# yanyan-li/Structure-SLAM-PointLine

Measured on AMD Instinct MI355X. Metric: front-end frames/sec (ORB+LSD extract+match) 640x480 @1000kp/200ln, higher is better.
Workload: dtype u8; 1 GPU; BASELINE configs[2]: 640x480 ORB(1000kp,8 levels)+LSD/LBD(<=200 lines) extract + Hamming match vs previous frame, inputs resident in HBM; batch_per_gpu=12288, global_batch=12288, unique_frames=64, streams=point branch and line branch on two HIP streams, parallelism=single GPU

## Files before the change

### structure-slam-pointline_amd/csrc/orb.hip

```cpp
#include "common.h"
#include "camera.h"
#include <cmath>
#include <algorithm>

using namespace sslam;

namespace {

constexpr int MAX_LEVELS = 16;
constexpr int MAX_ROOTS = 64;
constexpr int EDGE = 19;
constexpr int MINB = 16;
constexpr int HALF_PATCH = 15;

struct LevelInfo {
    int w, h, pitch;
    unsigned off;
    int cellBeg, nCells;
    int candOff, candCap;
    int nfeat;
    int selOff, selCap;
    int nIni;
    float hX;
    int W, H;
    float scale;
    float size;
    int tabX, tabY;
    float rcpGroups;
};

struct Plan {
    int nlevels;
    int nCellsFrame, candFrame, selFrame;
    unsigned blurPack0, blurPack1;
    const uint4* blurToep;
    int blurTapSum;
    size_t pyrFrame;
    const uint8_t* img0; size_t img0Stride; int img0Pitch;
    int maxCellW, maxCellH, maxCellsLevel, maxNodeCap;
    LevelInfo L[MAX_LEVELS];
};

struct CellInfo {
    short level, x0, y0, x1, y1;
    short pad;
    int candOff;
    unsigned magic, gmagic;
};

__device__ __forceinline__ const uint8_t* level_image(const Plan& P, const uint8_t* __restrict__ pyr, size_t pyrFrame, int b, int level, int& pitch) {
    if (level == 0 && P.img0) { pitch = P.img0Pitch; return P.img0 + (size_t)b * P.img0Stride; }
    pitch = P.L[level].pitch;
    return pyr + (size_t)b * pyrFrame + P.L[level].off;
}

__device__ const signed char kPat[1024] = {
#include "orb_pattern.inc"
};
__constant__ int kUmax[16];
typedef short s16x2 __attribute__((ext_vector_type(2)));
__device__ __forceinline__ s16x2 as_s16x2(unsigned v) { return __builtin_bit_cast(s16x2, v); }
__device__ __forceinline__ unsigned as_u32(s16x2 v) { return __builtin_bit_cast(unsigned, v); }
__constant__ unsigned kDiscMask[31 * 8];

__global__ void k_copy_level0(const uint8_t* __restrict__ in, size_t pitch, size_t imageStride,
                              uint8_t* __restrict__ pyr, size_t pyrFrame, int w, int h, int dpitch) {
    const int b = blockIdx.z;
    const int y = blockIdx.y;
    const int x = (blockIdx.x * blockDim.x + threadIdx.x) * 16;
    if (x >= w) return;
    const uint8_t* s = in + (size_t)b * imageStride + (size_t)y * pitch + x;
    uint8_t* d = pyr + (size_t)b * pyrFrame + (size_t)y * dpitch + x;
// ... 90 lines not shown
        cd = cd && ((r[k] < v - minTh) || (r[k + 8] < v - minTh));
    }
    if (!(cb || cd)) return 0;
    auto network = [&](int (&d)[16], int sg) -> int {
#pragma unroll
        for (int k = 0; k < 16; ++k) d[k] = (d[k] - v) ^ sg;
        const int d0 = d[0], d1 = d[1];
#pragma unroll
        for (int k = 0; k < 14; ++k) d[k] = min(min(d[k], d[k + 1]), d[k + 2]);
        d[14] = min(min(d[14], d[15]), d0);
        d[15] = min(min(d[15], d0), d1);
        int A = min(min(d[0], d[3]), d[6]);
#pragma unroll
        for (int k = 1; k < 16; ++k) A = max(A, min(min(d[k], d[(k + 3) & 15]), d[(k + 6) & 15]));
        return A - sg;
    };
    int best = max(0, network(r, cd ? -1 : 0));
    const bool both = cb && cd;
    if (__builtin_amdgcn_ballot_w64(both)) {
        const uint8_t* c2 = c;
        asm volatile("" : "+v"(c2));
        int q[16];
        q[0] = c2[3 * tp];      q[1] = c2[3 * tp + 1];   q[2] = c2[2 * tp + 2];   q[3] = c2[tp + 3];
        q[4] = c2[3];           q[5] = c2[-tp + 3];      q[6] = c2[-2 * tp + 2];  q[7] = c2[-3 * tp + 1];
        q[8] = c2[-3 * tp];     q[9] = c2[-3 * tp - 1];  q[10] = c2[-2 * tp - 2]; q[11] = c2[-tp - 3];
        q[12] = c2[-3];         q[13] = c2[tp - 3];      q[14] = c2[2 * tp - 2];  q[15] = c2[3 * tp - 1];
        const int b2 = network(q, 0);
        if (both) best = max(best, b2);
    }
    int s = best - 1;
    return s >= minTh ? s : 0;
}

constexpr int FAST_LIST_CAP = 832;

static inline int fast_tile_pitch(int maxW) { return (maxW + 6 + 3 + 7) & ~3; }
static inline int fast_score_pitch(int maxW) { return maxW + 1; }
static inline size_t fast_score_bytes(int maxW, int maxH) { return (((size_t)(maxH + 2) * fast_score_pitch(maxW) + 1) + 3) & ~(size_t)3; }
static inline size_t fast_lds_bytes(int maxW, int maxH) {
    return (size_t)(maxH + 6) * fast_tile_pitch(maxW) + fast_score_bytes(maxW, maxH) + sizeof(unsigned short) * FAST_LIST_CAP;
}

__global__ __launch_bounds__(64) void k_fast_cells(const uint8_t* __restrict__ pyr, size_t pyrFrame, Plan P,
                                                   const CellInfo* __restrict__ cells,
                                                   unsigned* __restrict__ cand, int* __restrict__ cellCount,
                                                   int iniTh, int minTh, int tileP, int scP) {
    extern __shared__ __align__(16) uint8_t lds[];
    const int b = blockIdx.y, per = gridDim.x >> 3;
    const int cellId = (((blockIdx.x & 7) + b) & 7) * per + (blockIdx.x >> 3);
    if (cellId >= P.nCellsFrame) return;
    const int lane = threadIdx.x;
    const CellInfo ci = cells[cellId];
    const LevelInfo& L = P.L[ci.level];
    const int cw = ci.x1 - ci.x0, ch = ci.y1 - ci.y0;
    uint8_t* tile = lds;
    uint8_t* sc = tile + (P.maxCellH + 6) * tileP;
    int pitch;
    const uint8_t* img = level_image(P, pyr, pyrFrame, b, ci.level, pitch);
    const int ax = (ci.x0 - 3) & ~3, off = (ci.x0 - 3) - ax;
    const int ndw = (off + cw + 6 + 3) >> 2, th = ch + 6;
    {
        const __amdgpu_buffer_rsrc_t rs = __builtin_amdgcn_make_buffer_rsrc((void*)(img + (size_t)(ci.y0 - 3) * pitch + ax), 0, 0x7FFFFFFF, 0x00020000);
        const int q0 = lane & 15;
        for (int ry = lane >> 4; ry < th; ry += 4) {
            const int rowOff = __mul24(ry, pitch);
            for (int q = q0; q < ndw; q += 16) ((unsigned*)(tile + ry * tileP))[q] = __builtin_amdgcn_raw_buffer_load_b32(rs, rowOff + 4 * q, 0, 0);
        }
    }
    for (int i = lane; i < (((ch + 2) * scP + 1 + 3) >> 2); i += 64) ((unsigned*)sc)[i] = 0;
    __syncthreads();
    const unsigned magic = ci.magic;
    unsigned short* clist = (unsigned short*)(sc + (((P.maxCellH + 2) * scP + 1 + 3) & ~3));
    int ncl = 0;
    bool dense = false;
    const int T0 = off + 3;
    const int gmin = T0 >> 2, ng = ((T0 + cw - 1) >> 2) - gmin + 1;
    const unsigned gmagic = ci.gmagic;
    const int nitems = ch * ng;
    for (int it0 = 0;;) {
        const s16x2 th2 = {(short)minTh, (short)minTh};
        int la = lane;
        asm volatile("" : "+v"(la));
        for (ncl = 0; it0 < nitems; it0 += 64) {
            const int it = it0 + la;
            unsigned flags = 0;
            int py = 0, g = 0;
            if (it < nitems) {
                py = (int)(__umul24((unsigned)it, gmagic) >> 19);
                g = gmin + (it - __mul24(py, ng));
                const int rowN = __mul24(py, tileP);
                const unsigned* rc = (const unsigned*)(tile + rowN + 3 * tileP) + g;
                const unsigned c1 = rc[0], c0 = rc[-1], c2 = rc[1];
                const unsigned n4 = ((const unsigned*)(tile + rowN))[g], s4 = ((const unsigned*)(tile + rowN + 6 * tileP))[g];
                unsigned res = 0;
#pragma unroll
                for (int h = 0; h < 2; ++h) {
                    const unsigned wsel = h == 0 ? 0x0c020c00u : 0x0c030c01u;
                    const s16x2 v = as_s16x2(__builtin_amdgcn_perm(0u, c1, wsel));
                    const s16x2 rn = as_s16x2(__builtin_amdgcn_perm(0u, n4, wsel)), rs = as_s16x2(__builtin_amdgcn_perm(0u, s4, wsel));
                    const s16x2 re = as_s16x2(__builtin_amdgcn_perm(c2, c1, h == 0 ? 0x0c050c03u : 0x0c060c04u)), rw = as_s16x2(__builtin_amdgcn_perm(c1, c0, h == 0 ? 0x0c030c01u : 0x0c040c02u));
                    const s16x2 vp = v + th2, vm = v - th2;
                    const s16x2 mxV = __builtin_elementwise_max(rn, rs), mnV = __builtin_elementwise_min(rn, rs);
                    const s16x2 mxH = __builtin_elementwise_max(re, rw), mnH = __builtin_elementwise_min(re, rw);
                    const unsigned bright = as_u32(vp - __builtin_elementwise_min(mxV, mxH));
                    const unsigned dark = as_u32(__builtin_elementwise_max(mnV, mnH) - vm);
                    const unsigned m = (bright | dark) & 0x80008000u;
                    res |= m >> (15 - h);
                }
                flags = (res & 3u) | ((res >> 14) & 12u);
                const int px0 = 4 * g - T0;
                flags &= (0xFu << max(0, -px0)) & (0xFu >> max(0, px0 + 4 - cw));
            }
            const int cntf = __popc(flags);
            const int incl = wave_incl_scan(cntf);
            const int tot = __builtin_amdgcn_readlane(incl, 63);
            if (ncl + tot > FAST_LIST_CAP) { dense = true; break; }
            int pos = ncl + incl - cntf;
            const int ibase = __mul24(py, cw) + 4 * g - T0;
#pragma unroll
            for (int k = 0; k < 4; ++k) if (flags & (1u << k)) clist[pos++] = (unsigned short)(ibase + k);
            ncl += tot;
        }
        __syncthreads();
        for (int j = lane; j < ncl; j += 64) {
            const int i = clist[j];
            const int py = (int)(__umul24((unsigned)i, magic) >> 19), px = i - __mul24(py, cw);
            const int s = fast_score16(tile + __mul24(py + 3, tileP) + (off + px + 3), tileP, minTh);
            if (s) sc[__mul24(py + 1, scP) + (px + 1)] = (uint8_t)s;
        }
        __syncthreads();
        if (it0 >= nitems) break;
    }
    auto keep_code = [&](const uint8_t* c) -> int {
        const int s = c[0];
        const int n0 = c[-1], n1 = c[1], n2 = c[-scP - 1], n3 = c[-scP], n4 = c[-scP + 1], n5 = c[scP - 1], n6 = c[scP], n7 = c[scP + 1];
        const int mx = max(max(max(n0, n1), max(n2, n3)), max(max(n4, n5), max(n6, n7)));
        return (s > mx) ? (s >= iniTh ? 2 : 1) : 0;
    };
    unsigned* out = cand + (size_t)b * P.candFrame + ci.candOff;
    int cnt20 = 0, n = 0;
    if (!dense) {
        for (int j0 = 0; j0 < ncl; j0 += 64) {
            const int j = j0 + lane;
            int cde = 0;
            if (j < ncl) {
                const int i = clist[j];
                const int py = (int)(__umul24((unsigned)i, magic) >> 19), px = i - __mul24(py, cw);
                cde = keep_code(sc + __mul24(py + 1, scP) + (px + 1));
                clist[j] = (unsigned short)(i | (cde << 13));
            }
            cnt20 += __popcll(__ballot(cde == 2));
        }
        __syncthreads();
        const int need = cnt20 > 0 ? 2 : 1;
        for (int j0 = 0; j0 < ncl; j0 += 64) {
            const int j = j0 + lane;
            int e = 0;
            if (j < ncl) e = clist[j];
            const bool keep = (e >> 13) >= need;
            unsigned long long m = __ballot(keep);
            if (keep) {
                const int i = e & 0x1FFF;
                const int py = (int)(__umul24((unsigned)i, magic) >> 19), px = i - __mul24(py, cw);
                int s = sc[__mul24(py + 1, scP) + (px + 1)];
                out[n + mbcnt(m)] = ((unsigned)s << 24) | ((unsigned)(ci.y0 + py - MINB) << 12) | (unsigned)(ci.x0 + px - MINB);
            }
            n += __popcll(m);
        }
    } else {
        const int npx = __mul24(ch, cw);
        for (int i0 = 0; i0 < npx; i0 += 64) {
            const int i = i0 + lane;
            int cde = 0;
            if (i < npx) {
                const int py = (int)(__umul24((unsigned)i, magic) >> 19), px = i - __mul24(py, cw);
                cde = keep_code(sc + __mul24(py + 1, scP) + (px + 1));
            }
            cnt20 += __popcll(__ballot(cde == 2));
        }
        const int need = cnt20 > 0 ? 2 : 1;
        for (int i0 = 0; i0 < npx; i0 += 64) {
            const int i = i0 + lane;
            bool keep = false;
            int py = 0, px = 0;
            if (i < npx) {
                py = (int)(__umul24((unsigned)i, magic) >> 19); px = i - __mul24(py, cw);
                keep = keep_code(sc + __mul24(py + 1, scP) + (px + 1)) >= need;
            }
            unsigned long long m = __ballot(keep);
            if (keep) {
                int s = sc[__mul24(py + 1, scP) + (px + 1)];
                out[n + mbcnt(m)] = ((unsigned)s << 24) | ((unsigned)(ci.y0 + py - MINB) << 12) | (unsigned)(ci.x0 + px - MINB);
            }
            n += __popcll(m);
        }
    }
    if (lane == 0) cellCount[(size_t)b * P.nCellsFrame + cellId] = n;
}

struct OctLds {
    int* pre;
    unsigned* box0;
    unsigned* box1;
    unsigned* start;
    int* count;
    unsigned* links;
    unsigned long long* expA;
    unsigned long long* expB;
};

#define NIL 0xFFFFu

__global__ __launch_bounds__(64) void k_octree(const unsigned* __restrict__ cand, const int* __restrict__ cellCount,
                                               const CellInfo* __restrict__ cells, unsigned* __restrict__ bufA,
                                               unsigned* __restrict__ bufB, unsigned* __restrict__ sel,
                                               int* __restrict__ selCount, Plan P, int NC, int NCp2) {
    extern __shared__ __align__(16) uint8_t lds[];
    const int b = blockIdx.y, level = (int)((blockIdx.x + b + (b >> 3) + (b >> 6) + (b >> 9)) % gridDim.x), lane = threadIdx.x;
    const LevelInfo& L = P.L[level];
    OctLds S;
    S.expA = (unsigned long long*)lds;
    S.expB = S.expA + NCp2;
    S.pre = (int*)(S.expB + NCp2);
    S.box0 = (unsigned*)(S.pre + P.maxCellsLevel + 1);
    S.box1 = S.box0 + NC;
    S.start = S.box1 + NC;
    S.count = (int*)(S.start + NC);
    S.links = (unsigned*)(S.count + NC);

    const int nc = L.nCells;
// ... 414 lines not shown
            default: w = 0xFFFFFFFFu; break;
        }
        ((unsigned*)kpOut)[((size_t)b * cap + outIdx) * 7 + lane] = w;
    }
}

__global__ __launch_bounds__(256) void k_orb_status(const int* __restrict__ selCount, int nlevels, int nframes, int cap, int* __restrict__ status) {
    __shared__ int cnt, first;
    if (threadIdx.x == 0) { cnt = 0; first = 0x7FFFFFFF; }
    __syncthreads();
    for (int b = threadIdx.x; b < nframes; b += 256) {
        int t = 0;
        for (int l = 0; l < nlevels; ++l) t += selCount[(size_t)b * nlevels + l];
        if (t > cap) { atomicAdd(&cnt, 1); atomicMin(&first, b); }
    }
    __syncthreads();
    if (threadIdx.x == 0) { status[0] = cnt; status[1] = first; status[2] = 0; status[3] = 0x7FFFFFFF; }
}

}

struct sslam_orb {
    sslam_ctx* ctx;
    int nfeatures, nlevels, iniTh, minTh;
    float scaleFactorF;
    double scaleFactor;
    std::vector<float> scale, invScale, sigma2, invSigma2;
    std::vector<int> perLevel;
    int umax[16];
    int planW = 0, planH = 0;
    Plan plan;
    const uint8_t* lastImg0 = nullptr; size_t lastImg0Pitch = 0, lastImg0Stride = 0; bool lastInPlace = false;
    std::vector<CellInfo> cells;
    std::vector<short> tabs;
    DevBuf dCells, dTabs, dPyr, dCellCount, dCand, dBufA, dBufB, dSel, dSelCount;
    DevBuf dImg, dKp, dDesc, dCounts;
    HostPinned hImg, hOut;
    int wsFrames = 0;
    int lastFrames = 0;
    int lastN = -1;
    bool constsUploaded = false;
    int blurVariant = 0;
    hipEvent_t gateEvent = nullptr;
    bool hasCamera = false; sslam_camera camera{};
    DevBuf dToep; int toepVariant = -1, toepSum = 0;
};

static inline int cvRoundF(float v) { return (int)lrintf(v); }

static std::vector<int> blur_taps_340(int n, double sigma) {
    std::vector<float> k(n); double sum = 0; const double s2 = -0.5 / (sigma * sigma);
    for (int i = 0; i < n; ++i) { const double x = i - (n - 1) * 0.5; k[i] = (float)std::exp(s2 * x * x); sum += k[i]; }
    sum = 1. / sum;
    std::vector<int> t(n);
    for (int i = 0; i < n; ++i) { k[i] = (float)(k[i] * sum); t[i] = (int)lrint((double)k[i] * 256.0); }
    return t;
}
static std::vector<int> blur_taps_q8(int n, double sigma) {
    std::vector<double> k(n);
    double sum = 0, s2 = -0.5 / (sigma * sigma);
    for (int i = 0; i < n; ++i) { double x = i - (n - 1) * 0.5; k[i] = std::exp(s2 * x * x); sum += k[i]; }
    std::vector<int> t(n);
    double err = 0; long isum = 0;
    for (int i = 0; i < n / 2; ++i) {
        double adj = k[i] / sum * 256.0 + err;
        int v = (int)lrint(adj);
        err = adj - v; t[i] = t[n - 1 - i] = v; isum += v;
    }
// ... 92 lines not shown
                o->tabs.push_back((short)cvRoundF((1.f - fx) * 2048));
                o->tabs.push_back((short)cvRoundF(fx * 2048));
                o->tabs.push_back(0);
            }
            L.tabY = (int)o->tabs.size() / 4;
            for (int dy = 0; dy < L.h; ++dy) {
                float fy = (float)((dy + 0.5) * sy_ - 0.5);
                int sy = (int)std::floor(fy);
                fy -= sy;
                o->tabs.push_back((short)sy);
                o->tabs.push_back((short)cvRoundF((1.f - fy) * 2048));
                o->tabs.push_back((short)cvRoundF(fy * 2048));
                o->tabs.push_back(0);
            }
            while ((o->tabs.size() / 4) % 4) o->tabs.insert(o->tabs.end(), 4, (short)0);
        }
    }
    {
        int lvl = 0;
        for (int l = 1; l < o->nlevels; ++l) if (P.L[l].selCap > P.L[lvl].selCap) lvl = l;
        int NC, NCp2; size_t lds;
        octree_lds(P, NC, NCp2, lds);
        if (NC > 0xFFFF) {
            set_error("nfeatures %d: level %d would give the quadtree %d node slots (limit %d: 16-bit slot numbers)", o->nfeatures, lvl, NC, 0xFFFF); return SSLAM_ERR_UNSUPPORTED;
        }
        int ldsMax = 0;
        SSLAM_HIP(hipDeviceGetAttribute(&ldsMax, hipDeviceAttributeMaxSharedMemoryPerBlock, o->ctx->device));
        if (lds > (size_t)ldsMax) {
            set_error("nfeatures %d: level %d (%d keypoints) needs %zu bytes of LDS for the quadtree, the device allows %d", o->nfeatures, lvl, P.L[lvl].nfeat, lds, ldsMax); return SSLAM_ERR_UNSUPPORTED;
        }
    }
    P.pyrFrame = (off + 16 + 255) & ~(size_t)255;
    P.nCellsFrame = (int)o->cells.size();
    P.candFrame = std::max(candOff, 1);
    P.selFrame = selOff;
    if (o->dCells.ensure(std::max<size_t>(o->cells.size(), 1) * sizeof(CellInfo)) != SSLAM_OK) return SSLAM_ERR_HIP;
    if (o->dTabs.ensure(std::max<size_t>(o->tabs.size(), 1) * sizeof(short)) != SSLAM_OK) return SSLAM_ERR_HIP;
    if (!o->cells.empty()) SSLAM_HIP(hipMemcpy(o->dCells.p, o->cells.data(), o->cells.size() * sizeof(CellInfo), hipMemcpyHostToDevice));
    if (!o->tabs.empty()) SSLAM_HIP(hipMemcpy(o->dTabs.p, o->tabs.data(), o->tabs.size() * sizeof(short), hipMemcpyHostToDevice));
    o->planW = w; o->planH = h;
    o->wsFrames = 0;
    return SSLAM_OK;
}

static int ensure_workspace(sslam_orb* o, int nframes) {
    if (nframes <= o->wsFrames) return SSLAM_OK;
    const Plan& P = o->plan;
    int rc;
    if ((rc = o->dPyr.ensure(P.pyrFrame * nframes))) return rc;
    if ((rc = o->dCellCount.ensure(sizeof(int) * (size_t)std::max(P.nCellsFrame, 1) * nframes))) return rc;
    if ((rc = o->dCand.ensure(sizeof(unsigned) * (size_t)P.candFrame * nframes))) return rc;
    if ((rc = o->dBufA.ensure(sizeof(unsigned) * (size_t)P.candFrame * nframes))) return rc;
    if ((rc = o->dBufB.ensure(sizeof(unsigned) * (size_t)P.candFrame * nframes))) return rc;
    if ((rc = o->dSel.ensure(sizeof(unsigned) * (size_t)P.selFrame * nframes))) return rc;
    if ((rc = o->dSelCount.ensure(sizeof(int) * (size_t)P.nlevels * nframes))) return rc;
    o->wsFrames = nframes;
    return SSLAM_OK;
}

extern "C" int sslam_orb_create(sslam_ctx* ctx, int nfeatures, float scaleFactor, int nlevels, int iniTh, int minTh, sslam_orb** out) {
    if (!ctx || !out || nlevels < 1 || nlevels > MAX_LEVELS || nfeatures < 0 || !(scaleFactor > 1.0f) || minTh < 1 || iniTh < minTh || iniTh > 255) {
        set_error("sslam_orb_create: invalid arguments"); return SSLAM_ERR_INVALID;
    }
    sslam_orb* o = new sslam_orb();
    o->ctx = ctx; o->nfeatures = nfeatures; o->nlevels = nlevels; o->iniTh = iniTh; o->minTh = minTh;
    o->scaleFactorF = scaleFactor; o->scaleFactor = (double)scaleFactor;
    o->scale.resize(nlevels); o->sigma2.resize(nlevels); o->invScale.resize(nlevels); o->invSigma2.resize(nlevels);
    o->scale[0] = 1.0f; o->sigma2[0] = 1.0f;
    for (int i = 1; i < nlevels; ++i) { o->scale[i] = (float)(o->scale[i - 1] * o->scaleFactor); o->sigma2[i] = o->scale[i] * o->scale[i]; }
    for (int i = 0; i < nlevels; ++i) { o->invScale[i] = 1.0f / o->scale[i]; o->invSigma2[i] = 1.0f / o->sigma2[i]; }
    o->perLevel.resize(nlevels);
    float factor = (float)(1.0f / o->scaleFactor);
    float nDesired = nfeatures * (1 - factor) / (1 - (float)std::pow((double)factor, (double)nlevels));
    int sum = 0;
    for (int l = 0; l < nlevels - 1; ++l) { o->perLevel[l] = cvRoundF(nDesired); sum += o->perLevel[l]; nDesired *= factor; }
    o->perLevel[nlevels - 1] = std::max(nfeatures - sum, 0);
    {
        int v, v0, vmax = (int)std::floor(HALF_PATCH * std::sqrt(2.f) / 2 + 1);
        int vmin = (int)std::ceil(HALF_PATCH * std::sqrt(2.f) / 2);
        const double hp2 = HALF_PATCH * HALF_PATCH;
        for (v = 0; v <= vmax; ++v) o->umax[v] = (int)lrint(std::sqrt(hp2 - v * v));
        for (v = HALF_PATCH, v0 = 0; v >= vmin; --v) { while (o->umax[v0] == o->umax[v0 + 1]) ++v0; o->umax[v] = v0; ++v0; }
    }
    *out = o;
    return SSLAM_OK;
}

extern "C" int sslam_orb_set_blur_variant(sslam_orb* o, int variant) {
    if (!o || (variant != 0 && variant != 1)) { set_error("sslam_orb_set_blur_variant: invalid arguments"); return SSLAM_ERR_INVALID; }
    std::lock_guard<std::recursive_mutex> lk(o->ctx->mu);
    o->blurVariant = variant;
    return SSLAM_OK;
}

extern "C" int sslam_orb_destroy(sslam_orb* o) {
    if (!o) return SSLAM_OK;
    (void)hipSetDevice(o->ctx->device);
    (void)hipStreamSynchronize(o->ctx->stream);
    DevBuf* bufs[] = {&o->dCells, &o->dTabs, &o->dPyr, &o->dCellCount, &o->dCand, &o->dBufA, &o->dBufB, &o->dSel, &o->dSelCount, &o->dImg, &o->dKp, &o->dDesc, &o->dCounts, &o->dToep};
    for (DevBuf* b : bufs) b->release();
    o->hImg.release(); o->hOut.release();
    delete o;
    return SSLAM_OK;
}

extern "C" int sslam_orb_get_scales(const sslam_orb* o, float* scale, float* inv_scale, float* sigma2, float* inv_sigma2, int32_t* per_level) {
    if (!o) return SSLAM_ERR_INVALID;
    for (int i = 0; i < o->nlevels; ++i) {
        if (scale) scale[i] = o->scale[i];
        if (inv_scale) inv_scale[i] = o->invScale[i];
        if (sigma2) sigma2[i] = o->sigma2[i];
        if (inv_sigma2) inv_sigma2[i] = o->invSigma2[i];
        if (per_level) per_level[i] = o->perLevel[i];
    }
    return SSLAM_OK;
}

extern "C" int sslam_orb_set_gate_event(sslam_orb* o, void* hip_event) {
    if (!o) { set_error("sslam_orb_set_gate_event: null handle"); return SSLAM_ERR_INVALID; }
    std::lock_guard<std::recursive_mutex> lk(o->ctx->mu);
    o->gateEvent = (hipEvent_t)hip_event;
    return SSLAM_OK;
}

extern "C" int sslam_orb_max_keypoints(const sslam_orb* o) {
    if (!o) return SSLAM_ERR_INVALID;
    int n = 0;
    for (int l = 0; l < o->nlevels; ++l) n += std::max(o->perLevel[l] + 3, 4 * 8 + 1);
    return n;
}

static int orb_prepare(sslam_orb* o, int w, int h, int nframes, hipStream_t st) {
// ... 31 lines not shown
                unsigned w = 0;
                for (int k = 0; k < 4; ++k) { const int u = 4 * m + k - 15; if (std::abs(u) <= o->umax[std::abs(r - 15)]) w |= 0xFFu << (8 * k); }
                mask[r * 8 + m] = w;
            }
        SSLAM_HIP(hipMemcpyToSymbol(HIP_SYMBOL(kDiscMask), mask, sizeof(mask)));
        o->constsUploaded = true;
    }
    if (nframes > o->wsFrames) { SSLAM_HIP(hipStreamSynchronize(st)); }
    return ensure_workspace(o, nframes);
}

static int orb_front(sslam_orb* o, Plan& P, const uint8_t* d_images, int w, int h, size_t pitch, size_t image_stride, int nframes, hipStream_t st) {
    uint8_t* pyr = o->dPyr.as<uint8_t>();
    const bool inPlace = ((uintptr_t)d_images & 3) == 0 && (pitch & 3) == 0 && (image_stride & 3) == 0 && pitch <= 0x7FFFFFFF &&
                         (pitch == (size_t)w || image_stride >= pitch * (size_t)h);
    P.img0 = inPlace ? d_images : nullptr; P.img0Stride = image_stride; P.img0Pitch = (int)pitch;
    o->lastImg0 = d_images; o->lastImg0Pitch = pitch; o->lastImg0Stride = image_stride; o->lastInPlace = inPlace;
    if (!inPlace) {
        dim3 blk(64), grd((w + 64 * 16 - 1) / (64 * 16), h, nframes);
        { sslam::ProfScope _ps(o->ctx, "k_copy_level0", st); hipLaunchKernelGGL(k_copy_level0, grd, blk, 0, st, d_images, pitch, image_stride, pyr, P.pyrFrame, w, h, P.L[0].pitch); }
    }
    for (int l = 1; l < P.nlevels; ++l) {
        const unsigned gx = (unsigned)((((P.L[l].w + 3) / 4) * P.L[l].h + 255) / 256);
        const int wantWgs = 32 * o->ctx->num_cus;
        const int gy = std::max(1, std::min(nframes, wantWgs / (int)std::max(gx, 1u)));
        dim3 blk(256), grd(gx, gy);
        const bool fromImage = l == 1 && inPlace;
        { sslam::ProfScope _ps(o->ctx, "k_resize", st);
          hipLaunchKernelGGL(k_resize, grd, blk, 0, st, fromImage ? d_images : pyr + P.L[l - 1].off, fromImage ? image_stride : P.pyrFrame, fromImage ? (int)pitch : P.L[l - 1].pitch, fromImage ? 1 : 0,
                             pyr, P.pyrFrame, P.L[l - 1], P.L[l], o->dTabs.as<short4>(), nframes); }
    }
    if (o->gateEvent) SSLAM_HIP(hipStreamWaitEvent(st, o->gateEvent, 0));
    if (P.nCellsFrame > 0) {
        const int tileP = fast_tile_pitch(P.maxCellW), scP = fast_score_pitch(P.maxCellW);
        const size_t lds = fast_lds_bytes(P.maxCellW, P.maxCellH);
        dim3 grd(8 * ((P.nCellsFrame + 7) / 8), nframes);
        { sslam::ProfScope _ps(o->ctx, "k_fast_cells", st); hipLaunchKernelGGL(k_fast_cells, grd, dim3(64), lds, st, pyr, P.pyrFrame, P, o->dCells.as<CellInfo>(), o->dCand.as<unsigned>(),
                           o->dCellCount.as<int>(), o->iniTh, o->minTh, tileP, scP); }
    }
    return SSLAM_OK;
}

static int orb_tail(sslam_orb* o, const Plan& P, int nframes, hipStream_t st, sslam_keypoint* d_kp, uint8_t* d_desc, int32_t* d_counts, int cap, size_t* octreeLdsOut) {
    uint8_t* pyr = o->dPyr.as<uint8_t>();
    {
        int NC, NCp2; size_t lds;
        octree_lds(P, NC, NCp2, lds);
        if (octreeLdsOut) *octreeLdsOut = lds;
        if (lds > 48 * 1024) SSLAM_HIP(hipFuncSetAttribute((const void*)k_octree, hipFuncAttributeMaxDynamicSharedMemorySize, (int)lds));
        dim3 grd(P.nlevels, nframes);
        { sslam::ProfScope _ps(o->ctx, "k_octree", st); hipLaunchKernelGGL(k_octree, grd, dim3(64), lds, st, o->dCand.as<unsigned>(), o->dCellCount.as<int>(), o->dCells.as<CellInfo>(),
                           o->dBufA.as<unsigned>(), o->dBufB.as<unsigned>(), o->dSel.as<unsigned>(), o->dSelCount.as<int>(), P, NC, NCp2); }
    }
    {
        dim3 grd(P.selFrame, nframes);
        { sslam::ProfScope _ps(o->ctx, "k_describe", st); hipLaunchKernelGGL(k_describe<false>, grd, dim3(64), 0, st, pyr, P.pyrFrame, P, o->dSel.as<unsigned>(), o->dSelCount.as<int>(),
                           d_kp, d_desc, d_counts, cap); }
    }
    SSLAM_HIP(hipGetLastError());
    o->lastFrames = nframes;
    return SSLAM_OK;
}

extern "C" int sslam_orb_extract_batch_dev(sslam_orb* o, const uint8_t* d_images, int w, int h, size_t pitch, size_t image_stride,
                                           int nframes, sslam_keypoint* d_kp, uint8_t* d_desc, int32_t* d_counts, int cap, void* stream_) {
    if (!o || !d_images || !d_kp || !d_desc || !d_counts || w <= 0 || h <= 0 || nframes <= 0 || cap <= 0 || pitch < (size_t)w) {
        set_error("sslam_orb_extract_batch_dev: invalid arguments"); return SSLAM_ERR_INVALID;
    }
    if (nframes > 1 && image_stride < pitch * (size_t)(h - 1) + (size_t)w) { set_error("sslam_orb_extract_batch_dev: the frames overlap (image_stride < pitch * (h - 1) + w)"); return SSLAM_ERR_INVALID; }
    std::lock_guard<std::recursive_mutex> lk(o->ctx->mu);
    SSLAM_HIP(hipSetDevice(o->ctx->device));
// ... 192 lines not shown
    SSLAM_HIP(hipMemcpyAsync(kp_out, o->dKp.p, sizeof(sslam_keypoint) * rows, hipMemcpyDeviceToHost, st));
    SSLAM_HIP(hipMemcpyAsync(desc_out, o->dDesc.p, 32 * rows, hipMemcpyDeviceToHost, st));
    SSLAM_HIP(hipMemcpyAsync(counts_out, o->dCounts.p, sizeof(int32_t) * (size_t)nframes, hipMemcpyDeviceToHost, st));
    SSLAM_HIP(hipMemcpyAsync(level_counts_out, o->dSelCount.p, sizeof(int32_t) * (size_t)nl * nframes, hipMemcpyDeviceToHost, st));
    SSLAM_HIP(hipStreamSynchronize(st));
    return SSLAM_OK;
}
#endif

int sslam_frame_from_device(sslam_ctx* ctx, int kind, const void* d_feats, const uint8_t* d_desc, int n, const float bounds[4], sslam_frame** out);
extern "C" int sslam_frame_from_orb(sslam_orb* o, const float bounds[4], sslam_frame** out) {
    if (!o || !bounds || !out) { set_error("sslam_frame_from_orb: invalid arguments"); return SSLAM_ERR_INVALID; }
    if (o->lastN < 0) { set_error("sslam_frame_from_orb: no sslam_orb_extract call to snapshot"); return SSLAM_ERR_INVALID; }
    std::lock_guard<std::recursive_mutex> lk(o->ctx->mu);
    int rc = sslam_frame_from_device(o->ctx, 0, o->dKp.p, o->dDesc.as<uint8_t>(), o->lastN, bounds, out);
    if (rc || !o->hasCamera || o->camera.k1 == 0.0f || o->lastN == 0) return rc;
    sslam_keypoint* d = (*out)->feats.as<sslam_keypoint>();
    hipError_t e = hipSuccess;
    if ((rc = undistort_launch(o->ctx, o->camera, d, nullptr, o->lastN, 1, o->lastN, d, o->ctx->stream)) == SSLAM_OK &&
        (e = hipStreamSynchronize(o->ctx->stream)) != hipSuccess) { set_error("sslam_frame_from_orb: %s", hipGetErrorString(e)); rc = SSLAM_ERR_HIP; }
    if (rc) { sslam_frame_destroy(*out); *out = nullptr; }
    return rc;
}

extern "C" int sslam_orb_set_camera(sslam_orb* o, const sslam_camera* cam) {
    if (!o || (cam && (cam->fx == 0.0f || cam->fy == 0.0f))) { set_error("sslam_orb_set_camera: invalid arguments"); return SSLAM_ERR_INVALID; }
    std::lock_guard<std::recursive_mutex> lk(o->ctx->mu);
    o->hasCamera = cam != nullptr;
    o->camera = cam ? *cam : sslam_camera{};
    return SSLAM_OK;
}

extern "C" sslam_ctx* sslam_orb_context(sslam_orb* o) { return o ? o->ctx : nullptr; }
```

Baseline: 83440 frames/s.

## Process up to three adjacent FAST cells per workgroup as a horizontal strip

FAST detection now runs over strips that merge up to three horizontally adjacent cells of the same level into one 64-lane workgroup. This shares the halo rows and columns between neighbouring cells and cuts the number of workgroups per frame. Per-cell non-max suppression borders, the threshold fallback and output offsets are kept by ballots over each cell's column range. Tile staging now uses direct buffer-to-LDS loads with a flattened row/dword index. The cost is extra per-pixel bookkeeping, a larger candidate list capacity in LDS, and fewer workgroups for latency hiding.

```diff
diff --git a/structure-slam-pointline_amd/csrc/fast_strips.h b/structure-slam-pointline_amd/csrc/fast_strips.h
--- /dev/null
+++ b/structure-slam-pointline_amd/csrc/fast_strips.h
@@ -0,0 +1,67 @@
+#pragma once
+#include <cstdint>
+#include <vector>
+
+namespace sslam_fast {
+
+constexpr int FAST_STRIP_K = 3;
+constexpr int FAST_LIST_CAP = 832 * FAST_STRIP_K;
+constexpr int FAST_IDX_BITS = 13;
+constexpr int FAST_MAX_PIXELS = 1 << FAST_IDX_BITS;
+constexpr int FAST_DIV_SHIFT = 20;
+
+struct StripInfo {
+    short level, x0, y0, x1, y1;
+    short nc;
+    short wc;
+    short pad;
+    int cellBeg;
+    unsigned magic, gmagic;
+    unsigned smagic;
+};
+
+inline unsigned fast_div_magic(int w) { return (1u << FAST_DIV_SHIFT) / (unsigned)w + 1; }
+
+inline bool fast_div_exact(int w, int n) {
+    if (w < 1 || n < 1) return false;
+    const uint64_t m = fast_div_magic(w), e = m * (uint64_t)w - (1u << FAST_DIV_SHIFT);
+    return m < (1u << 24) && (uint64_t)n <= (1u << 24) && (uint64_t)(n - 1) * m < (1ull << 32) && (uint64_t)(n - 1) * e < (1u << FAST_DIV_SHIFT);
+}
+
+inline int fast_groups(int x0, int w) {
+    const int T0 = ((x0 - 3) & 3) + 3;
+    return ((T0 + w - 1) >> 2) - (T0 >> 2) + 1;
+}
+
+inline int fast_stage_dwords(int x0, int w) { return (((x0 - 3) & 3) + w + 6 + 3) >> 2; }
+
+inline bool fast_strip_fits(int x0, int w, int h) {
+    const int ng = fast_groups(x0, w);
+    return w * h <= FAST_MAX_PIXELS && fast_div_exact(w, w * h) && fast_div_exact(ng, ng * h) && fast_div_exact(fast_stage_dwords(x0, w), 65);
+}
+
+template <class Cell>
+inline bool fast_build_strips(const Cell* cells, int n, std::vector<StripInfo>& out) {
+    out.clear();
+    for (int k = 0; k < n; ++k) {
+        const Cell& c = cells[k];
+        const int h = c.y1 - c.y0;
+        bool extend = false;
+        if (!out.empty()) {
+            const StripInfo& s = out.back();
+            extend = s.level == c.level && s.y0 == c.y0 && s.y1 == c.y1 && s.x1 == c.x0 && s.nc < FAST_STRIP_K && s.cellBeg + s.nc == k &&
+                     s.x1 - s.x0 == s.nc * s.wc && c.x1 - c.x0 <= s.wc && fast_strip_fits(s.x0, c.x1 - s.x0, h);
+        }
+        if (extend) { out.back().x1 = c.x1; out.back().nc++; }
+        else {
+            if (!fast_strip_fits(c.x0, c.x1 - c.x0, h)) return false;
+            StripInfo s{};
+            s.level = c.level; s.x0 = c.x0; s.y0 = c.y0; s.x1 = c.x1; s.y1 = c.y1; s.nc = 1; s.wc = (short)(c.x1 - c.x0); s.cellBeg = k;
+            out.push_back(s);
+        }
+    }
+    for (StripInfo& s : out) { s.magic = fast_div_magic(s.x1 - s.x0); s.gmagic = fast_div_magic(fast_groups(s.x0, s.x1 - s.x0)); s.smagic = fast_div_magic(fast_stage_dwords(s.x0, s.x1 - s.x0)); }
+    return true;
+}
+
+}
diff --git a/structure-slam-pointline_amd/csrc/orb.hip b/structure-slam-pointline_amd/csrc/orb.hip
--- a/structure-slam-pointline_amd/csrc/orb.hip
+++ b/structure-slam-pointline_amd/csrc/orb.hip
@@ -1,9 +1,11 @@
 #include "common.h"
 #include "camera.h"
+#include "fast_strips.h"
 #include <cmath>
 #include <algorithm>
 
 using namespace sslam;
+using sslam_fast::StripInfo; using sslam_fast::FAST_STRIP_K; using sslam_fast::FAST_LIST_CAP; using sslam_fast::FAST_IDX_BITS; using sslam_fast::FAST_DIV_SHIFT;
 
 namespace {
 
@@ -38,6 +40,7 @@
     size_t pyrFrame;
     const uint8_t* img0; size_t img0Stride; int img0Pitch;
     int maxCellW, maxCellH, maxCellsLevel, maxNodeCap;
+    int nStripsFrame, maxStripW;
     LevelInfo L[MAX_LEVELS];
 };
 
@@ -194,50 +197,62 @@
     return s >= minTh ? s : 0;
 }
 
-constexpr int FAST_LIST_CAP = 832;
-
 static inline int fast_tile_pitch(int maxW) { return (maxW + 6 + 3 + 7) & ~3; }
-static inline int fast_score_pitch(int maxW) { return maxW + 1; }
-static inline size_t fast_score_bytes(int maxW, int maxH) { return (((size_t)(maxH + 2) * fast_score_pitch(maxW) + 1) + 3) & ~(size_t)3; }
+static inline size_t fast_score_bytes(int maxW, int maxH) { return (((size_t)(maxH + 2) * (maxW + 1) + 1) + 3) & ~(size_t)3; }
 static inline size_t fast_lds_bytes(int maxW, int maxH) {
     return (size_t)(maxH + 6) * fast_tile_pitch(maxW) + fast_score_bytes(maxW, maxH) + sizeof(unsigned short) * FAST_LIST_CAP;
 }
 
+#ifdef SSLAM_FAST_CYCLES
+__device__ unsigned long long g_fastCycles[8];
+#define FAST_CLK(k) do { const unsigned long long t_ = __builtin_readcyclecounter(); clk[k] += t_ - tPrev; tPrev = t_; } while (0)
+#else
+#define FAST_CLK(k) do {} while (0)
+#endif
+
 __global__ __launch_bounds__(64) void k_fast_cells(const uint8_t* __restrict__ pyr, size_t pyrFrame, Plan P,
-                                                   const CellInfo* __restrict__ cells,
+                                                   const StripInfo* __restrict__ strips, const CellInfo* __restrict__ cells,
                                                    unsigned* __restrict__ cand, int* __restrict__ cellCount,
-                                                   int iniTh, int minTh, int tileP, int scP) {
+                                                   int iniTh, int minTh, int tileMaxP) {
     extern __shared__ __align__(16) uint8_t lds[];
     const int b = blockIdx.y, per = gridDim.x >> 3;
-    const int cellId = (((blockIdx.x & 7) + b) & 7) * per + (blockIdx.x >> 3);
-    if (cellId >= P.nCellsFrame) return;
+    const int stripId = (((blockIdx.x & 7) + b) & 7) * per + (blockIdx.x >> 3);
+    if (stripId >= P.nStripsFrame) return;
+#ifdef SSLAM_FAST_CYCLES
+    unsigned long long clk[5] = {0, 0, 0, 0, 0}, tPrev = __builtin_readcyclecounter();
+#endif
     const int lane = threadIdx.x;
-    const CellInfo ci = cells[cellId];
-    const LevelInfo& L = P.L[ci.level];
-    const int cw = ci.x1 - ci.x0, ch = ci.y1 - ci.y0;
+    const StripInfo si = strips[stripId];
+    const int sw = si.x1 - si.x0, ch = si.y1 - si.y0, wc = si.wc;
+    const int scP = sw + 1;
     uint8_t* tile = lds;
-    uint8_t* sc = tile + (P.maxCellH + 6) * tileP;
+    uint8_t* sc = tile + (P.maxCellH + 6) * tileMaxP;
     int pitch;
-    const uint8_t* img = level_image(P, pyr, pyrFrame, b, ci.level, pitch);
-    const int ax = (ci.x0 - 3) & ~3, off = (ci.x0 - 3) - ax;
-    const int ndw = (off + cw + 6 + 3) >> 2, th = ch + 6;
+    const uint8_t* img = level_image(P, pyr, pyrFrame, b, si.level, pitch);
+    const int ax = (si.x0 - 3) & ~3, off = (si.x0 - 3) - ax;
+    const int ndw = (off + sw + 6 + 3) >> 2, th = ch + 6;
+    const int tileP = 4 * ndw;
     {
-        const __amdgpu_buffer_rsrc_t rs = __builtin_amdgcn_make_buffer_rsrc((void*)(img + (size_t)(ci.y0 - 3) * pitch + ax), 0, 0x7FFFFFFF, 0x00020000);
-        const int q0 = lane & 15;
-        for (int ry = lane >> 4; ry < th; ry += 4) {
-            const int rowOff = __mul24(ry, pitch);
-            for (int q = q0; q < ndw; q += 16) ((unsigned*)(tile + ry * tileP))[q] = __builtin_amdgcn_raw_buffer_load_b32(rs, rowOff + 4 * q, 0, 0);
+        const __amdgpu_buffer_rsrc_t rs = __builtin_amdgcn_make_buffer_rsrc((void*)(img + (size_t)(si.y0 - 3) * pitch + ax), 0, 0x7FFFFFFF, 0x00020000);
+        const int rstep = (int)((64u * si.smagic) >> FAST_DIV_SHIFT), qstep = 64 - rstep * ndw;
+        int ry = (int)(__umul24((unsigned)lane, si.smagic) >> FAST_DIV_SHIFT), q = lane - __mul24(ry, ndw);
+        const int ndwords = th * ndw;
+        for (int base = 0; base < ndwords; base += 64) {
+            if (ry < th) __builtin_amdgcn_raw_ptr_buffer_load_lds(rs, (__attribute__((address_space(3))) void*)(tile + 4 * base), 4, __mul24(ry, pitch) + 4 * q, 0, 0, 0);
+            ry += rstep; q += qstep;
+            if (q >= ndw) { q -= ndw; ++ry; }
         }
     }
     for (int i = lane; i < (((ch + 2) * scP + 1 + 3) >> 2); i += 64) ((unsigned*)sc)[i] = 0;
     __syncthreads();
-    const unsigned magic = ci.magic;
-    unsigned short* clist = (unsigned short*)(sc + (((P.maxCellH + 2) * scP + 1 + 3) & ~3));
+    FAST_CLK(0);
+    const unsigned magic = si.magic;
+    unsigned short* clist = (unsigned short*)(sc + (((P.maxCellH + 2) * (P.maxStripW + 1) + 1 + 3) & ~3));
     int ncl = 0;
     bool dense = false;
     const int T0 = off + 3;
-    const int gmin = T0 >> 2, ng = ((T0 + cw - 1) >> 2) - gmin + 1;
-    const unsigned gmagic = ci.gmagic;
+    const int gmin = T0 >> 2, ng = ((T0 + sw - 1) >> 2) - gmin + 1;
+    const unsigned gmagic = si.gmagic;
     const int nitems = ch * ng;
     for (int it0 = 0;;) {
         const s16x2 th2 = {(short)minTh, (short)minTh};
@@ -248,7 +263,7 @@
             unsigned flags = 0;
             int py = 0, g = 0;
             if (it < nitems) {
-                py = (int)(__umul24((unsigned)it, gmagic) >> 19);
+                py = (int)(__umul24((unsigned)it, gmagic) >> FAST_DIV_SHIFT);
                 g = gmin + (it - __mul24(py, ng));
                 const int rowN = __mul24(py, tileP);
                 const unsigned* rc = (const unsigned*)(tile + rowN + 3 * tileP) + g;
@@ -271,93 +286,121 @@
                 }
                 flags = (res & 3u) | ((res >> 14) & 12u);
                 const int px0 = 4 * g - T0;
-                flags &= (0xFu << max(0, -px0)) & (0xFu >> max(0, px0 + 4 - cw));
+                flags &= (0xFu << max(0, -px0)) & (0xFu >> max(0, px0 + 4 - sw));
             }
             const int cntf = __popc(flags);
             const int incl = wave_incl_scan(cntf);
             const int tot = __builtin_amdgcn_readlane(incl, 63);
             if (ncl + tot > FAST_LIST_CAP) { dense = true; break; }
             int pos = ncl + incl - cntf;
-            const int ibase = __mul24(py, cw) + 4 * g - T0;
+            const int ibase = __mul24(py, sw) + 4 * g - T0;
 #pragma unroll
             for (int k = 0; k < 4; ++k) if (flags & (1u << k)) clist[pos++] = (unsigned short)(ibase + k);
             ncl += tot;
         }
         __syncthreads();
+        FAST_CLK(1);
         for (int j = lane; j < ncl; j += 64) {
             const int i = clist[j];
-            const int py = (int)(__umul24((unsigned)i, magic) >> 19), px = i - __mul24(py, cw);
+            const int py = (int)(__umul24((unsigned)i, magic) >> FAST_DIV_SHIFT), px = i - __mul24(py, sw);
             const int s = fast_score16(tile + __mul24(py + 3, tileP) + (off + px + 3), tileP, minTh);
             if (s) sc[__mul24(py + 1, scP) + (px + 1)] = (uint8_t)s;
         }
         __syncthreads();
+        FAST_CLK(2);
         if (it0 >= nitems) break;
     }
-    auto keep_code = [&](const uint8_t* c) -> int {
+    auto first_col = [&](int px) -> bool {
+        bool f = px == 0;
+#pragma unroll
+        for (int k = 1; k < FAST_STRIP_K; ++k) f = f || px == k * wc;
+        return f;
+    };
+    auto last_col = [&](int px) -> bool {
+        bool f = false;
+#pragma unroll
+        for (int k = 1; k < FAST_STRIP_K; ++k) f = f || px == k * wc - 1;
+        return f;
+    };
+    auto in_cell = [&](const unsigned long long (&ge)[FAST_STRIP_K], int k) -> unsigned long long {
+        return k == 0 ? (FAST_STRIP_K > 1 ? ~ge[1] : ~0ull) : (k == FAST_STRIP_K - 1 ? ge[k] : ge[k] & ~ge[k + 1]);
+    };
+    auto keep_code = [&](const uint8_t* c, bool first, bool last) -> int {
         const int s = c[0];
         const int n0 = c[-1], n1 = c[1], n2 = c[-scP - 1], n3 = c[-scP], n4 = c[-scP + 1], n5 = c[scP - 1], n6 = c[scP], n7 = c[scP + 1];
-        const int mx = max(max(max(n0, n1), max(n2, n3)), max(max(n4, n5), max(n6, n7)));
+        const int mxL = first ? 0 : max(max(n0, n2), n5), mxR = last ? 0 : max(max(n1, n4), n7);
+        const int mx = max(max(mxL, mxR), max(n3, n6));
         return (s > mx) ? (s >= iniTh ? 2 : 1) : 0;
     };
-    unsigned* out = cand + (size_t)b * P.candFrame + ci.candOff;
-    int cnt20 = 0, n = 0;
-    if (!dense) {
-        for (int j0 = 0; j0 < ncl; j0 += 64) {
-            const int j = j0 + lane;
-            int cde = 0;
-            if (j < ncl) {
-                const int i = clist[j];
-                const int py = (int)(__umul24((unsigned)i, magic) >> 19), px = i - __mul24(py, cw);
-                cde = keep_code(sc + __mul24(py + 1, scP) + (px + 1));
-                clist[j] = (unsigned short)(i | (cde << 13));
-            }
-            cnt20 += __popcll(__ballot(cde == 2));
-        }
-        __syncthreads();
-        const int need = cnt20 > 0 ? 2 : 1;
-        for (int j0 = 0; j0 < ncl; j0 += 64) {
-            const int j = j0 + lane;
-            int e = 0;
-            if (j < ncl) e = clist[j];
-            const bool keep = (e >> 13) >= need;
-            unsigned long long m = __ballot(keep);
-            if (keep) {
-                const int i = e & 0x1FFF;
-                const int py = (int)(__umul24((unsigned)i, magic) >> 19), px = i - __mul24(py, cw);
-                int s = sc[__mul24(py + 1, scP) + (px + 1)];
-                out[n + mbcnt(m)] = ((unsigned)s << 24) | ((unsigned)(ci.y0 + py - MINB) << 12) | (unsigned)(ci.x0 + px - MINB);
-            }
-            n += __popcll(m);
-        }
-    } else {
-        const int npx = __mul24(ch, cw);
-        for (int i0 = 0; i0 < npx; i0 += 64) {
-            const int i = i0 + lane;
-            int cde = 0;
-            if (i < npx) {
-                const int py = (int)(__umul24((unsigned)i, magic) >> 19), px = i - __mul24(py, cw);
-                cde = keep_code(sc + __mul24(py + 1, scP) + (px + 1));
-            }
-            cnt20 += __popcll(__ballot(cde == 2));
-        }
-        const int need = cnt20 > 0 ? 2 : 1;
-        for (int i0 = 0; i0 < npx; i0 += 64) {
-            const int i = i0 + lane;
-            bool keep = false;
-            int py = 0, px = 0;
-            if (i < npx) {
-                py = (int)(__umul24((unsigned)i, magic) >> 19); px = i - __mul24(py, cw);
-                keep = keep_code(sc + __mul24(py + 1, scP) + (px + 1)) >= need;
-            }
-            unsigned long long m = __ballot(keep);
-            if (keep) {
-                int s = sc[__mul24(py + 1, scP) + (px + 1)];
-                out[n + mbcnt(m)] = ((unsigned)s << 24) | ((unsigned)(ci.y0 + py - MINB) << 12) | (unsigned)(ci.x0 + px - MINB);
-            }
-            n += __popcll(m);
-        }
-    }
-    if (lane == 0) cellCount[(size_t)b * P.nCellsFrame + cellId] = n;
+    const int nvis = dense ? __mul24(ch, sw) : ncl;
+    int cnt20[FAST_STRIP_K], n[FAST_STRIP_K], co[FAST_STRIP_K];
+#pragma unroll
+    for (int k = 0; k < FAST_STRIP_K; ++k) { cnt20[k] = 0; n[k] = 0; co[k] = k < si.nc ? cells[si.cellBeg + k].candOff : 0; }
+    for (int j0 = 0; j0 < nvis; j0 += 64) {
+        const int j = j0 + lane;
+        int cde = 0, px = 0;
+        if (j < nvis) {
+            const int i = dense ? j : (int)clist[j];
+            const int py = (int)(__umul24((unsigned)i, magic) >> FAST_DIV_SHIFT);
+            px = i - __mul24(py, sw);
+            cde = keep_code(sc + __mul24(py + 1, scP) + (px + 1), first_col(px), last_col(px));
+            if (!dense) clist[j] = (unsigned short)(i | (cde << FAST_IDX_BITS));
+        }
+        const unsigned long long m2 = __ballot(cde == 2);
+        unsigned long long ge[FAST_STRIP_K] = {};
+#pragma unroll
+        for (int k = 1; k < FAST_STRIP_K; ++k) ge[k] = __ballot(px >= k * wc);
+#pragma unroll
+        for (int k = 0; k < FAST_STRIP_K; ++k) cnt20[k] += __popcll(m2 & in_cell(ge, k));
+    }
+    __syncthreads();
+    FAST_CLK(3);
+    unsigned* out = cand + (size_t)b * P.candFrame;
+    for (int j0 = 0; j0 < nvis; j0 += 64) {
+        const int j = j0 + lane;
+        int cde = 0, py = 0, px = 0;
+        if (j < nvis) {
+            if (dense) {
+                py = (int)(__umul24((unsigned)j, magic) >> FAST_DIV_SHIFT); px = j - __mul24(py, sw);
+                cde = keep_code(sc + __mul24(py + 1, scP) + (px + 1), first_col(px), last_col(px));
+            } else {
+                const int e = clist[j], i = e & ((1 << FAST_IDX_BITS) - 1);
+                cde = e >> FAST_IDX_BITS;
+                py = (int)(__umul24((unsigned)i, magic) >> FAST_DIV_SHIFT); px = i - __mul24(py, sw);
+            }
+        }
+        const unsigned long long m2 = __ballot(cde == 2), m1 = __ballot(cde >= 1);
+        unsigned long long ge[FAST_STRIP_K] = {};
+#pragma unroll
+        for (int k = 1; k < FAST_STRIP_K; ++k) ge[k] = __ballot(px >= k * wc);
+        int pos = 0;
+        unsigned long long any = 0;
+#pragma unroll
+        for (int k = 0; k < FAST_STRIP_K; ++k) {
+            const unsigned long long m = (cnt20[k] > 0 ? m2 : m1) & in_cell(ge, k);
+            const int at = co[k] + n[k] + mbcnt(m);
+            if (__builtin_amdgcn_inverse_ballot_w64(m)) pos = at;
+            n[k] += __popcll(m);
+            any |= m;
+        }
+        if (__builtin_amdgcn_inverse_ballot_w64(any)) {
+            const int s = sc[__mul24(py + 1, scP) + (px + 1)];
+            out[pos] = ((unsigned)s << 24) | ((unsigned)(si.y0 + py - MINB) << 12) | (unsigned)(si.x0 + px - MINB);
+        }
+    }
+    if (lane < si.nc) {
+        int nk = n[0];
+#pragma unroll
+        for (int k = 1; k < FAST_STRIP_K; ++k) nk = lane == k ? n[k] : nk;
+        cellCount[(size_t)b * P.nCellsFrame + si.cellBeg + lane] = nk;
+    }
+#ifdef SSLAM_FAST_CYCLES
+    FAST_CLK(4);
+    if (lane == 0) {
+        for (int k = 0; k < 5; ++k) atomicAdd(&g_fastCycles[k], clk[k]);
+        atomicAdd(&g_fastCycles[5], 1ull);
+    }
+#endif
 }
 
 struct OctLds {
@@ -838,8 +881,9 @@
     Plan plan;
     const uint8_t* lastImg0 = nullptr; size_t lastImg0Pitch = 0, lastImg0Stride = 0; bool lastInPlace = false;
     std::vector<CellInfo> cells;
+    std::vector<StripInfo> strips;
     std::vector<short> tabs;
-    DevBuf dCells, dTabs, dPyr, dCellCount, dCand, dBufA, dBufB, dSel, dSelCount;
+    DevBuf dCells, dStrips, dTabs, dPyr, dCellCount, dCand, dBufA, dBufB, dSel, dSelCount;
     DevBuf dImg, dKp, dDesc, dCounts;
     HostPinned hImg, hOut;
     int wsFrames = 0;
@@ -998,11 +1042,16 @@
     }
     P.pyrFrame = (off + 16 + 255) & ~(size_t)255;
     P.nCellsFrame = (int)o->cells.size();
+    if (!sslam_fast::fast_build_strips(o->cells.data(), (int)o->cells.size(), o->strips)) { set_error("image size %dx%d: a FAST cell is larger than k_fast_cells' index range", w, h); return SSLAM_ERR_UNSUPPORTED; }
+    P.nStripsFrame = (int)o->strips.size();
+    for (const StripInfo& s : o->strips) P.maxStripW = std::max(P.maxStripW, s.x1 - s.x0);
     P.candFrame = std::max(candOff, 1);
     P.selFrame = selOff;
     if (o->dCells.ensure(std::max<size_t>(o->cells.size(), 1) * sizeof(CellInfo)) != SSLAM_OK) return SSLAM_ERR_HIP;
+    if (o->dStrips.ensure(std::max<size_t>(o->strips.size(), 1) * sizeof(StripInfo)) != SSLAM_OK) return SSLAM_ERR_HIP;
     if (o->dTabs.ensure(std::max<size_t>(o->tabs.size(), 1) * sizeof(short)) != SSLAM_OK) return SSLAM_ERR_HIP;
     if (!o->cells.empty()) SSLAM_HIP(hipMemcpy(o->dCells.p, o->cells.data(), o->cells.size() * sizeof(CellInfo), hipMemcpyHostToDevice));
+    if (!o->strips.empty()) SSLAM_HIP(hipMemcpy(o->dStrips.p, o->strips.data(), o->strips.size() * sizeof(StripInfo), hipMemcpyHostToDevice));
     if (!o->tabs.empty()) SSLAM_HIP(hipMemcpy(o->dTabs.p, o->tabs.data(), o->tabs.size() * sizeof(short), hipMemcpyHostToDevice));
     o->planW = w; o->planH = h;
     o->wsFrames = 0;
@@ -1063,7 +1112,7 @@
     if (!o) return SSLAM_OK;
     (void)hipSetDevice(o->ctx->device);
     (void)hipStreamSynchronize(o->ctx->stream);
-    DevBuf* bufs[] = {&o->dCells, &o->dTabs, &o->dPyr, &o->dCellCount, &o->dCand, &o->dBufA, &o->dBufB, &o->dSel, &o->dSelCount, &o->dImg, &o->dKp, &o->dDesc, &o->dCounts, &o->dToep};
+    DevBuf* bufs[] = {&o->dCells, &o->dStrips, &o->dTabs, &o->dPyr, &o->dCellCount, &o->dCand, &o->dBufA, &o->dBufB, &o->dSel, &o->dSelCount, &o->dImg, &o->dKp, &o->dDesc, &o->dCounts, &o->dToep};
     for (DevBuf* b : bufs) b->release();
     o->hImg.release(); o->hOut.release();
     delete o;
@@ -1161,11 +1210,11 @@
     }
     if (o->gateEvent) SSLAM_HIP(hipStreamWaitEvent(st, o->gateEvent, 0));
     if (P.nCellsFrame > 0) {
-        const int tileP = fast_tile_pitch(P.maxCellW), scP = fast_score_pitch(P.maxCellW);
-        const size_t lds = fast_lds_bytes(P.maxCellW, P.maxCellH);
-        dim3 grd(8 * ((P.nCellsFrame + 7) / 8), nframes);
-        { sslam::ProfScope _ps(o->ctx, "k_fast_cells", st); hipLaunchKernelGGL(k_fast_cells, grd, dim3(64), lds, st, pyr, P.pyrFrame, P, o->dCells.as<CellInfo>(), o->dCand.as<unsigned>(),
-                           o->dCellCount.as<int>(), o->iniTh, o->minTh, tileP, scP); }
+        const int tileP = fast_tile_pitch(P.maxStripW);
+        const size_t lds = fast_lds_bytes(P.maxStripW, P.maxCellH);
+        dim3 grd(8 * ((P.nStripsFrame + 7) / 8), nframes);
+        { sslam::ProfScope _ps(o->ctx, "k_fast_cells", st); hipLaunchKernelGGL(k_fast_cells, grd, dim3(64), lds, st, pyr, P.pyrFrame, P, o->dStrips.as<StripInfo>(), o->dCells.as<CellInfo>(),
+                           o->dCand.as<unsigned>(), o->dCellCount.as<int>(), o->iniTh, o->minTh, tileP); }
     }
     return SSLAM_OK;
 }
@@ -1424,3 +1473,12 @@
 }
 
 extern "C" sslam_ctx* sslam_orb_context(sslam_orb* o) { return o ? o->ctx : nullptr; }
+
+#ifdef SSLAM_FAST_CYCLES
+extern "C" int sslam_testing_orb_fast_cycles(unsigned long long* out8, int reset) {
+    SSLAM_HIP(hipDeviceSynchronize());
+    if (out8) SSLAM_HIP(hipMemcpyFromSymbol(out8, HIP_SYMBOL(g_fastCycles), sizeof(unsigned long long) * 8));
+    if (reset) { const unsigned long long z[8] = {0, 0, 0, 0, 0, 0, 0, 0}; SSLAM_HIP(hipMemcpyToSymbol(HIP_SYMBOL(g_fastCycles), z, sizeof(z))); }
+    return SSLAM_OK;
+}
+#endif
```

Measured after the change: 84270 frames/s, median of 6. 1.0% higher.
